# MP-Gadget/MP-Gadget

Hardware: AMD Instinct MI355X
Metric: particle-updates/sec (gravity force step: PM + tree build + short-range walk) (higher is better)
Workload: dtype f64; 1 GPU; 256^3 DM-only TreePM force step, Nmesh=512, s_zel ICs, all particles active, relative opening criterion (ErrTolForceAcc 0.002), TreeRcut 6, Asmth 1.5; particles=16777216, nmesh=512, parallelism=1 GPU

## Files before the change

### include/mpgadget_hip.h

```cpp
#ifndef MPGADGET_HIP_H
#define MPGADGET_HIP_H

#include <stddef.h>
#include <stdint.h>

#ifdef __cplusplus
extern "C" {
#endif

typedef struct mpg_engine mpg_engine;

int mpg_engine_create(mpg_engine **out, int device);
void mpg_engine_destroy(mpg_engine *eng);
const char *mpg_last_error(void);
const char *mpg_version(void);
const char *mpg_build_stamp(void);
int mpg_engine_set_stream(mpg_engine *eng, void *hip_stream);
void *mpg_engine_get_stream(mpg_engine *eng);
int mpg_engine_synchronize(mpg_engine *eng);

typedef struct mpg_gravshort_tree_params {
    double ErrTolForceAcc;
    double BHOpeningAngle;
    double MaxBHOpeningAngle;
// ... 185 lines not shown
    double density_in_phys_cgs;
    double uu_in_cgs;
    double tt_in_s;
    double units_rho_crit_baryon;
    double sfr_MinGasTemp;
    double temp_to_u;
    double HIReionTemp;
    int test_network_maxiter;
} mpg_cooling_params;
typedef struct mpg_cooling_step {
    mpg_uvbg uvbg;
    double long_mean_free_path_heating;
    double lastred[47];
    double redshift;
    double helium;
} mpg_cooling_step;
typedef struct mpg_cooling_arrays {
    const double *density;
    double *entropy;
    double *ne;
    double *sfr;
    const double *metallicity;
    const uint8_t *heiii_ionized;
    const uint8_t *tb_hydro;
} mpg_cooling_arrays;
int mpg_set_cooling_params(mpg_engine *eng, const mpg_cooling_params *par);
int mpg_set_metal_cooling_table(mpg_engine *eng, int nz, const double *zbins, int nnh, const double *nhbins, int nt, const double *tbins,
                                const double *rate);
int mpg_dev_cooling(mpg_engine *eng, const mpg_cooling_arrays *A, const mpg_sph_times *T, const mpg_cooling_step *step, const int *d_active,
                    int64_t nactive);
int mpg_cooling(mpg_engine *eng, const mpg_particle_view *pv, double BoxSize, const mpg_cooling_arrays *A, const mpg_sph_times *T,
                const mpg_cooling_step *step, const int *ActiveParticle, int64_t NumActiveParticle);
int mpg_resident_sph_cooling(mpg_engine *eng, const mpg_particle_view *pv, const mpg_sph_times *T, const mpg_cooling_step *step,
                             const int *ActiveParticle, int64_t NumActiveParticle, double *ne, const double *metallicity,
                             const uint8_t *heiii_ionized);
int mpg_dev_cooling_state(mpg_engine *eng, int64_t n, const double *d_rho, const double *d_u, double *d_ne_inout, double *d_lambdanet,
                          double *d_temp, double *d_nh0, const mpg_cooling_step *step);
int mpg_cooling_get_stats(mpg_engine *eng, int64_t stats[6]);
int mpg_cooling_export(mpg_engine *eng, int64_t n, int32_t *evaluations);

typedef struct mpg_tree_stats {
    int64_t NumParticles;
    int64_t numnodes;
    int64_t numleaves;
    int32_t maxlevel;
    double root_mass, root_cofm[3], root_hmax;
} mpg_tree_stats;
int mpg_tree_get_stats(mpg_engine *eng, mpg_tree_stats *st);
int mpg_tree_export(mpg_engine *eng, int32_t *level, double *center, double *len, double *cofm, double *mass, double *hmax,
                    int32_t *sibling, int32_t *pstart, int32_t *pcount);
int mpg_tree_export_order(mpg_engine *eng, int32_t *order);
int mpg_walk_get_counters(mpg_engine *eng, int64_t counters[10]);
int mpg_walk_get_f32_stats(mpg_engine *eng, int64_t out[2]);
typedef struct mpg_phase_times {
    float pm_deposit, pm_fft, pm_transfer, pm_readout, pm_total;
    float tree_keys, tree_sort, tree_nodes, tree_moments, tree_total;
    float walk;
    int32_t walk_launches;
} mpg_phase_times;
int mpg_get_phase_times(mpg_engine *eng, mpg_phase_times *t);
int mpg_set_instrumentation(mpg_engine *eng, int timing, int counters);
int mpg_walk_events_collect(mpg_engine *eng, double *total_ms, int *count);
int mpg_walk_events_collect2(mpg_engine *eng, double *total_ms, int *count, double *lists_ms, double *eval_ms, int *count_split);
const int *mpg_dev_tree_order(mpg_engine *eng);
int mpg_grav_short_pair(mpg_engine *eng, const mpg_particle_view *pv, const int *ActiveParticle, int64_t NumActiveParticle, double Rcut,
                        double rho0);
int mpg_dev_grav_short_pair(mpg_engine *eng, const int *d_active, int64_t nactive, double Rcut, double *d_accel, double *d_potential,
                            double rho0);

#define MPG_TIMEBINS 46
typedef struct mpg_kick_factors_s {
    double gravkick[MPG_TIMEBINS + 1];
    double hydrokick[MPG_TIMEBINS + 1];
    double dt_entr[MPG_TIMEBINS + 1];
    unsigned char bin_active[MPG_TIMEBINS + 1];
    double atime, MaxGasVel;
} mpg_kick_factors;
int mpg_dev_drift_all_particles(mpg_engine *eng, int64_t n, double *d_pos, const double *d_vel, const unsigned char *d_type,
                                const unsigned char *d_flags, double *d_hsml, const double *d_dthsml, double ddrift, double BoxSize,
                                const double random_shift[3]);
int mpg_dev_apply_pm_half_kick(mpg_engine *eng, int64_t n, double *d_vel, const double *d_gravpm, const unsigned char *d_flags, double Fgravkick);
int mpg_dev_apply_half_kick(mpg_engine *eng, int64_t n, const int *d_active, int64_t nactive, double *d_vel, const double *d_gravaccel,
                            const unsigned char *d_type, const unsigned char *d_flags, const unsigned char *d_tb_grav,
                            const unsigned char *d_tb_hydro, const double *d_hydroaccel, double *d_entropy, const double *d_dtentropy,
                            const mpg_kick_factors *K);
int mpg_dev_apply_hydro_half_kick(mpg_engine *eng, int64_t n, const int *d_active, int64_t nactive, double *d_vel, const unsigned char *d_type,
                                  const unsigned char *d_flags, const unsigned char *d_tb_hydro, const double *d_hydroaccel, double *d_entropy,
                                  const double *d_dtentropy, const mpg_kick_factors *K);

int mpg_dev_timestep_gravity_dloga(mpg_engine *eng, int64_t n, const double *d_gravaccel, const double *d_gravpm, double atime, double hubble,
                                   double ErrTolIntAccuracy, double *d_dloga);

int mpg_dev_timestep_hydro_dloga(mpg_engine *eng, int64_t n, const unsigned char *d_type, const double *d_hsml, const double *d_dthsml,
                                 const double *d_maxsignalvel, const unsigned char *d_bh_mintimebin, const double *dloga_for_bin, double atime,
                                 double hubble, double CourantFac, double *d_dloga, unsigned char *d_titype);

typedef struct {
    int64_t nsync;
    const double *loga;
} mpg_timeline;
typedef struct {
    int mintimebin, maxtimebin, mingravtimebin;
    int64_t Ti_kick[MPG_TIMEBINS + 1];
    int64_t Ti_lastactivedrift[MPG_TIMEBINS + 1];
    int64_t Ti_Current;
    int64_t PM_length, PM_start, PM_kick;
// ... 214 lines not shown
                             void **d_new_cols);
int mpg_dist_use_decomposition(mpg_dist *d, double BoxSize, double margin, int La);
int mpg_dist_domain_maintain(mpg_dist *d, int64_t n, const double *d_pos, const unsigned char *d_garbage, double BoxSize, int64_t *n_leaving);
int mpg_dist_set_domain(mpg_dist *d, double BoxSize, const mpg_topnode *TopNodes, int NTopNodes, const int *leaf_task, int NTopLeaves,
                        double margin, int La);
int mpg_dist_gravity_step(mpg_dist *d, int64_t n_own, const double *d_pos, const float *d_mass, const double *d_oldacc,
                          const double *d_prev_accel, double *d_accel, double *d_gravpm, double *d_potential, double rho0);
int mpg_dist_dev_gravpm_force(mpg_dist *d, int64_t n_own, const double *d_pos, const float *d_mass, double *d_gravpm, double *d_potential);
int mpg_dist_dev_set_types(mpg_dist *d, int64_t n_own, const uint8_t *d_type);
int mpg_dist_dev_set_garbage(mpg_dist *d, int64_t n_own, const unsigned char *d_garbage);
int mpg_dist_dev_force_tree_build(mpg_dist *d, int64_t n_own, const double *d_pos, const float *d_mass);
int mpg_dist_dev_grav_short_tree(mpg_dist *d, const double *d_oldacc, const double *d_prev_accel, const double *d_gravpm, double *d_accel,
                                 double *d_potential, double rho0);
int mpg_dist_dev_grav_short_tree_active_tree(mpg_dist *d, int64_t n_act, const double *d_pos, const float *d_mass, const double *d_oldacc,
                                             double *d_accel, double *d_potential, double rho0);
int mpg_dist_grav_short_tree_active_tree(mpg_dist *d, const mpg_particle_view *pv, const int *ActiveParticle, int64_t NumActiveParticle,
                                         double (*AccelStore)[3], double rho0);
int mpg_dist_dev_grav_short_tree_active(mpg_dist *d, const int *d_active, int64_t nactive, const double *d_oldacc, const double *d_prev_accel,
                                        const double *d_gravpm, double *d_accel, double *d_potential, double rho0);
int mpg_dist_dev_density(mpg_dist *d, int64_t n_own, const uint8_t *d_type, const mpg_sph_arrays *A, const mpg_sph_times *T, int update_hsml,
                         int DoEgyDensity);
int mpg_dist_dev_hydro_force(mpg_dist *d, int64_t n_own, const mpg_sph_arrays *A, const mpg_sph_times *T);
int mpg_dist_dev_density_active(mpg_dist *d, int64_t n_own, const uint8_t *d_type, const mpg_sph_arrays *A, const mpg_sph_times *T,
                                const int *d_active, int64_t nactive, int update_hsml, int DoEgyDensity);
int mpg_dist_dev_hydro_force_active(mpg_dist *d, int64_t n_own, const mpg_sph_arrays *A, const mpg_sph_times *T, const int *d_active,
                                    int64_t nactive);
int mpg_dist_dev_fof_fof(mpg_dist *d, int64_t n_own, const double *d_pos, const float *d_mass, const uint8_t *d_type, const uint64_t *d_id,
                         const double *d_vel, const mpg_fof_params *par, int64_t *d_grnr, int64_t *ngroups_total, int64_t *ngroups_here);
int mpg_dist_fof_groups(mpg_dist *d, const mpg_fof_groups *out);
int mpg_dist_gravpm_force(mpg_dist *d, const mpg_particle_view *pv);
int mpg_dist_force_tree_full(mpg_dist *d, const mpg_particle_view *pv);
int mpg_dist_grav_short_tree(mpg_dist *d, const mpg_particle_view *pv, double (*AccelStore)[3], double rho0);
int mpg_dist_grav_short_tree_active(mpg_dist *d, const mpg_particle_view *pv, const int *ActiveParticle, int64_t NumActiveParticle,
                                    double (*AccelStore)[3], double rho0);
int mpg_dist_set_sph_options(mpg_dist *d, int BlackHoleOn);
double mpg_dist_last_max_hsml(mpg_dist *d);
int mpg_dist_domain_set_maxpart(mpg_dist *d, int64_t MaxPart);
int mpg_dist_gravpm_get_powerspectrum(mpg_dist *d, double BoxSize_in_MPC, double *kk, double *Power, int64_t *Nmodes, int *nonzero);
int mpg_dist_potential_planes(mpg_dist *d, int64_t n_own, const double *d_pos, const float *d_mass, const uint8_t *d_type,
                              const unsigned char *d_flags, double BoxSize, const mpg_plane_params *params, double *d_planes, int64_t *npart);
int mpg_dist_density(mpg_dist *d, const mpg_particle_view *pv, const mpg_sph_arrays *A, const mpg_sph_times *T, const int *ActiveParticle,
                     int64_t NumActiveParticle, int update_hsml, int DoEgyDensity);
int mpg_dist_hydro_force(mpg_dist *d, const mpg_particle_view *pv, const mpg_sph_arrays *A, const mpg_sph_times *T, const int *ActiveParticle,
                         int64_t NumActiveParticle);
const float *mpg_dist_walk_cost(mpg_dist *d);
int mpg_dist_get_stats(mpg_dist *d, int64_t stats[8]);
int mpg_dist_get_times(mpg_dist *d, double ms[8]);
int mpg_dev_force_tree_set_min_leaf_level(mpg_engine *eng, int level);

int mpg_set_walk_threshold(mpg_engine *eng, int thresh);
int mpg_set_walk_split_mode(mpg_engine *eng, int overlap, int chunks_per_wave);
int mpg_set_walk_list_capacity(mpg_engine *eng, int cap);
int mpg_set_walk_offsets64(mpg_engine *eng, int on);
int mpg_set_walk_variant(mpg_engine *eng, int variant);
int mpg_get_walk_choice(mpg_engine *eng, int *variant, int *list_capacity, unsigned *last_overflow);

#ifdef __cplusplus
}
#endif
#endif
```

### mp-gadget_amd/csrc/engine.hip

```cpp
#include "engine_internal.h"
#include <cstdio>

static thread_local std::string g_err;
std::string &mpg_err_slot() { return g_err; }

extern "C" {

const char *mpg_last_error(void) { return g_err.c_str(); }
const char *mpg_version(void) { return "mpgadget_hip 0.1 (gfx950; TreePM gravity: PM + tree + short-range walk)"; }

int mpg_engine_create(mpg_engine **out, int device)
{
    API_BEGIN
    MPG_CHECK(out != nullptr, "mpg_engine_create: null output pointer");
    int ndev = 0;
    hipError_t e = hipGetDeviceCount(&ndev);
    if(e != hipSuccess || ndev <= 0)
        fail(__FILE__, __LINE__, "mpg_engine_create: no HIP device available (this engine has no CPU path)");
    MPG_CHECK(device >= 0 && device < ndev, "mpg_engine_create: bad device index");
    MPG_HIP(hipSetDevice(device));
    mpg_engine *eng = new mpg_engine();
    eng->device = device;
    MPG_HIP(hipStreamCreateWithFlags(&eng->stream, hipStreamNonBlocking));
    eng->own_stream = true;
// ... 1747 lines not shown
            cofm[3 * j + 0] = m[j].x;
            cofm[3 * j + 1] = m[j].y;
            cofm[3 * j + 2] = m[j].z;
        }
        if(mass)
            mass[j] = m[j].m;
        if(hmax)
            hmax[j] = hm.empty() ? 0.0 : hm[j];
    }
    API_END
}

int mpg_tree_export_order(mpg_engine *eng, int32_t *order)
{
    API_BEGIN
    MPG_CHECK(eng && order, "null argument");
    MPG_CHECK(eng->tree_allocated, "no tree");
    MPG_HIP(hipSetDevice(eng->device));
    MPG_HIP(hipStreamSynchronize(eng->stream));
    MPG_HIP(hipMemcpy(order, eng->tree.idx_b.p, eng->tree.npart * sizeof(int32_t), hipMemcpyDeviceToHost));
    API_END
}

int mpg_walk_get_counters(mpg_engine *eng, int64_t counters[10])
{
    API_BEGIN
    MPG_CHECK(eng && counters, "null argument");
    MPG_HIP(hipSetDevice(eng->device));
    MPG_HIP(hipStreamSynchronize(eng->stream));
    unsigned long long c[16] = {0};
    MPG_HIP(hipMemcpy(c, eng->counters.p, 16 * sizeof(unsigned long long), hipMemcpyDeviceToHost));
    counters[0] = (int64_t)c[0];
    counters[1] = (int64_t)c[1];
    counters[2] = (int64_t)c[2];
    counters[3] = eng->last_targets;
    for(int k = 0; k < 6; k++)
        counters[4 + k] = (int64_t)c[3 + k];
    API_END
}

int mpg_walk_get_f32_stats(mpg_engine *eng, int64_t out[2])
{
    API_BEGIN
    MPG_CHECK(eng && out, "null argument");
    MPG_HIP(hipSetDevice(eng->device));
    MPG_HIP(hipStreamSynchronize(eng->stream));
    unsigned long long c[16] = {0};
    MPG_HIP(hipMemcpy(c, eng->counters.p, 16 * sizeof(unsigned long long), hipMemcpyDeviceToHost));
    out[0] = (int64_t)c[12];
    out[1] = (int64_t)c[13];
    API_END
}

int mpg_get_phase_times(mpg_engine *eng, mpg_phase_times *t)
{
    API_BEGIN
    MPG_CHECK(eng && t, "null argument");
    *t = eng->timer.t;
    API_END
}

int mpg_set_instrumentation(mpg_engine *eng, int timing, int counters)
{
    API_BEGIN
    MPG_CHECK(eng, "null engine");
    eng->timer.enabled = timing != 0;
    eng->count = counters != 0;
    API_END
}

int mpg_walk_events_collect2(mpg_engine *eng, double *total_ms, int *count, double *lists_ms, double *eval_ms, int *count_split)
{
    API_BEGIN
    MPG_CHECK(eng && total_ms && count, "null argument");
    MPG_HIP(hipSetDevice(eng->device));
    MPG_HIP(hipStreamSynchronize(eng->stream));
    double tot = 0, tl = 0, te = 0;
    int c = 0, cs = 0;
    for(size_t k = 0; k < eng->walk_events.size(); k++) {
        auto &ev = eng->walk_events[k];
        float ms = 0;
        MPG_HIP(hipEventSynchronize(ev.second));
        MPG_HIP(hipEventElapsedTime(&ms, ev.first, ev.second));
        tot += ms;
        c++;
        if(hipEvent_t mid = k < eng->walk_mid.size() ? eng->walk_mid[k] : nullptr) {
            float a = 0, b = 0;
            MPG_HIP(hipEventElapsedTime(&a, ev.first, mid));
            MPG_HIP(hipEventElapsedTime(&b, mid, ev.second));
            tl += a;
            te += b;
            cs++;
            eng->free_mid.push_back(mid);
        }
        eng->free_events.push_back(ev);
    }
    eng->walk_events.clear();
    eng->walk_mid.clear();
    *total_ms = tot;
    *count = c;
    if(lists_ms)
        *lists_ms = tl;
    if(eval_ms)
        *eval_ms = te;
    if(count_split)
        *count_split = cs;
    API_END
}

int mpg_walk_events_collect(mpg_engine *eng, double *total_ms, int *count)
{
    return mpg_walk_events_collect2(eng, total_ms, count, nullptr, nullptr, nullptr);
}

const int *mpg_dev_tree_order(mpg_engine *eng) { return (eng && eng->tree_allocated) ? (const int *)eng->tree.idx_b.p : nullptr; }

int mpg_set_walk_split_mode(mpg_engine *eng, int overlap, int chunks_per_wave)
{
    API_BEGIN
    MPG_CHECK(eng && chunks_per_wave >= 0 && chunks_per_wave <= 1024, "bad argument");
    eng->w3.split_overlap = overlap != 0;
    eng->w3.split_chunks_per_wave = chunks_per_wave;
    API_END
}

int mpg_set_walk_offsets64(mpg_engine *eng, int on)
{
    API_BEGIN
    MPG_CHECK(eng, "null engine");
    eng->w3.split_offsets64 = on != 0;
    API_END
}

int mpg_set_walk_threshold(mpg_engine *eng, int thresh)
{
    API_BEGIN
    MPG_CHECK(eng, "null engine");
    eng->walk_thresh = thresh;
    API_END
}

int mpg_set_walk_list_capacity(mpg_engine *eng, int cap)
{
    API_BEGIN
    MPG_CHECK(eng && cap >= 16 && cap <= 65536, "walk list capacity must be in [16, 65536]");
    eng->w3.cap = cap;
    eng->w3.split_cap = (cap + 7) / 8 * 8;
    API_END
}

int mpg_get_walk_choice(mpg_engine *eng, int *variant, int *list_capacity, unsigned *last_overflow)
{
    API_BEGIN
    MPG_CHECK(eng && variant, "null argument");
    *variant = eng->walk_variant ? eng->walk_variant : eng->walk_choice;
    if(list_capacity)
        *list_capacity = eng->w3.split_cap;
    if(last_overflow)
        *last_overflow = eng->w3.split_last_overflow;
    API_END
}

int mpg_set_walk_variant(mpg_engine *eng, int variant)
{
    API_BEGIN
    MPG_CHECK(eng && (variant == 0 || variant == 1 || variant == 4 || variant == 6), "walk variant must be 0 (auto), 1, 4 or 6");
    eng->walk_variant = variant;
    eng->walk_choice = 0;
    API_END
}

}
```

### mp-gadget_amd/csrc/grav_walk.h

```cpp
#pragma once
#include "mpg_common.h"

namespace mpg {

struct WalkIO {
    int64_t ntargets = 0;
    const int *targets = nullptr;
    const double *pos = nullptr;
    const float *mass = nullptr;
    const double *oldacc = nullptr;
    const double *prev_accel = nullptr;
    const double *gravpm = nullptr;
    double *accel = nullptr;
    double *potential = nullptr;
    const float *tab_force = nullptr;
    const float *tab_pot = nullptr;
    unsigned long long *counters = nullptr;
    int list_prio = 0, eval_prio = 0;
    float *cost = nullptr;
};

void launch_grav_walk(const TreeView &tv, const GravParams &gp, const WalkIO &io, bool want_pot, bool count, bool fastwrap, int thresh,
                      hipStream_t st);

struct WalkScratch {
    DevBuf<int2> list;
    DevBuf<unsigned> ctr;
    int cap = 512;
    int num_cu = 0;
    DevBuf<unsigned> split_lists;
    DevBuf<int2> split_counts;
    DevBuf<int> split_ovf;
    int split_cap = 512;
    int split_slice = 1 << 25;
    size_t split_bytes = 80ull << 30;
    unsigned split_last_overflow = 0, split_last_maxlen = 0;
    bool split_overlap = false;
    bool split_offsets64 = false;
    int split_chunks_per_wave = 1;
    hipEvent_t ev_mid = nullptr;
    bool mid_recorded = false;
    hipEvent_t ev_before_eval = nullptr;
    hipStream_t split_stream = nullptr;
    hipEvent_t ev_lists[2] = {nullptr, nullptr}, ev_eval[2] = {nullptr, nullptr}, ev_begin = nullptr;
    ~WalkScratch()
    {
        for(hipEvent_t e : {ev_lists[0], ev_lists[1], ev_eval[0], ev_eval[1], ev_begin})
            if(e)
                (void)hipEventDestroy(e);
        if(split_stream)
            (void)hipStreamDestroy(split_stream);
    }
};
void launch_grav_walk_coop(const TreeView &tv, const GravParams &gp, const WalkIO &io, bool want_pot, bool count, bool fastwrap,
                           WalkScratch &ws, hipStream_t st);
void launch_grav_walk_split(const TreeView &tv, const GravParams &gp, const WalkIO &io, bool want_pot, bool count, bool fastwrap, WalkScratch &ws,
                            hipStream_t st);
void launch_grav_short_pair(const TreeView &tv, const GravParams &gp, const WalkIO &io, double rcut_abs, bool want_pot, unsigned *d_err,
                            hipStream_t st);
unsigned walk_coop_error(WalkScratch &ws, hipStream_t st);

}
```

### mp-gadget_amd/csrc/grav_walk_split.hip

```cpp
#include "grav_walk.h"
#include <cstdlib>
#include <cstring>
#include <cstdio>
#include <type_traits>

namespace mpg {

namespace {

constexpr int EVAL_BLOCKS = 4;
constexpr int LIST_BLOCKS = 6;

__device__ __forceinline__ double rsqrt_nr(double x)
{
    const double y = __builtin_amdgcn_rsq(x);
    const double e = fma(-(x * y), y, 1.0);
    return fma(y * e, fma(e, 0.375, 0.5), y);
}

template <unsigned long long BITS>
__device__ __forceinline__ double scalar_literal()
{
    unsigned lo, hi;
    asm volatile("s_mov_b32 %0, %2\n\ts_mov_b32 %1, %3" : "=s"(lo), "=s"(hi) : "i"((unsigned)(BITS & 0xffffffffull)), "i"((unsigned)(BITS >> 32)));
// ... 581 lines not shown
        if(tvalid) {
            const bool overflow = (overflowed >> lane) & 1u;
            if(io.cost)
                io.cost[ci] = (float)(8 * (overflow ? cap : nl) + nn + 3 * (nl + nn));
            if(overflow) {
                counts[rel] = make_int2(-1, 0);
                ovf[atomicAdd(&ctl[0], 1u)] = ci;
            }
            else {
                counts[rel] = make_int2(nl | (wrapped ? (1 << 30) : 0), nn);
                if((unsigned)(nl + nn) > ctl[2])
                    atomicMax(&ctl[2], (unsigned)(nl + nn));
            }
        }
        if(COUNT) {
#pragma unroll
            for(int t = 0; t < 8; t++)
                if(!((overflowed >> t) & 1u)) {
                    n_pp += c_pp[t];
                    if(lane == 0) {
                        n_vis += T.c_vis[t];
                        n_used += T.c_used[t];
                        n_le += (unsigned)T.nleaf[t];
                        n_se += (unsigned)T.nnode[t];
                    }
                }
        }
    }
    if(COUNT) {
        unsigned long long c0 = n_pp, c1 = n_vis, c2 = n_used, c3 = lane == 0 ? st_a : 0u, c4 = lane == 0 ? st_al : 0u;
        for(int off = 32; off > 0; off >>= 1) {
            c0 += __shfl_down(c0, off);
            c1 += __shfl_down(c1, off);
            c2 += __shfl_down(c2, off);
            c3 += __shfl_down(c3, off);
            c4 += __shfl_down(c4, off);
        }
        if(lane == 0) {
            atomicAdd(&io.counters[5], n_le);
            atomicAdd(&io.counters[6], n_se);
            atomicAdd(&io.counters[0], c0);
            atomicAdd(&io.counters[1], c1);
            atomicAdd(&io.counters[2], c2);
            atomicAdd(&io.counters[3], c3);
            atomicAdd(&io.counters[4], c4);
            if(F32 && n_amb)
                atomicAdd(&io.counters[12], (unsigned long long)n_amb);
            if(F32 && n_f32w)
                atomicAdd(&io.counters[13], (unsigned long long)n_f32w);
        }
    }
}

constexpr int RING_STRIDE = 17;

template <bool POT, bool WRAP, bool O32>
__device__ __forceinline__ void eval_lists(const TreeView &tv, const GravParams &gp, const unsigned *__restrict__ L, const int cap, const int nleaf,
                                           const int nnode, const int s, const int gshift, const double px,
                                           const double py, const double pz, const double *__restrict__ s_wtab, unsigned *__restrict__ ring_g,
                                           double &ax, double &ay, double &az, double &pot)
{
    const unsigned empty = (unsigned)tv.nnodes;
    const unsigned s32 = (unsigned)s * 32u;
#define MPG_LOAD(EJ, SV)                                                                        \
    {                                                                                           \
        const unsigned ej_ = (EJ);                                                              \
        if(O32)                                                                                 \
            SV = *(const Src4 *)((const char *)tv.srcL + (size_t)((ej_ << 8) + s32));           \
        else                                                                                    \
            SV = tv.srcL[(size_t)ej_ * 8 + (size_t)s];                                          \
    }
#define MPG_EVAL(SV)                                                              \
    {                                                                             \
        __builtin_amdgcn_sched_barrier(0);                                        \
        double dx_ = SV.x - px, dy_ = SV.y - py, dz_ = SV.z - pz;                 \
        if(WRAP) {                                                                \
            dx_ = nearest_img(dx_, gp.box, gp.invbox);                            \
            dy_ = nearest_img(dy_, gp.box, gp.invbox);                            \
            dz_ = nearest_img(dz_, gp.box, gp.invbox);                            \
        }                                                                         \
        pair_force<POT>(SV, dx_, dy_, dz_, gp, s_wtab, ax, ay, az, pot);           \
        asm volatile("" : "+v"(ax), "+v"(ay), "+v"(az), "+v"(pot));               \
        __builtin_amdgcn_sched_barrier(0);                                        \
    }
    {
        const unsigned ls = (unsigned)((gshift >> 3) * cap + s);
#define MPG_LEAF_AT(E0) (ls + (unsigned)(E0))
        __builtin_amdgcn_wave_barrier();
        ring_g[s] = (s < nleaf) ? ld<true>(L, MPG_LEAF_AT(0)) : empty;
        unsigned ent_n = (8 + s < nleaf) ? ld<true>(L, MPG_LEAF_AT(8)) : empty;
        __builtin_amdgcn_wave_barrier();
        unsigned eb = ring_g[1];
        Src4 A, B;
        MPG_LOAD(ring_g[0], A);
        int wmax = nleaf;
        for(int off = 8; off < 64; off <<= 1)
            wmax = max(wmax, __shfl_xor(wmax, off));
        wmax = __builtin_amdgcn_readfirstlane(wmax);
        Src4 Cq = A;
        MPG_LOAD(eb, B);
        int staged = 1;
#pragma unroll 1
        for(int e = 0; e < wmax; e += 3) {
            if(e + 4 >= 8 * staged) {
                ring_g[(staged & 1) * 8 + s] = ent_n;
                ent_n = ((staged + 1) * 8 + s < nleaf) ? ld<true>(L, MPG_LEAF_AT((staged + 1) * 8)) : empty;
                staged++;
                __builtin_amdgcn_wave_barrier();
            }
            const unsigned e2 = ring_g[(e + 2) & 15], e3 = ring_g[(e + 3) & 15], e4 = ring_g[(e + 4) & 15];
            MPG_LOAD(e2, Cq);
            MPG_EVAL(A);
            MPG_LOAD(e3, A);
            MPG_EVAL(B);
            MPG_LOAD(e4, B);
            MPG_EVAL(Cq);
        }
    }
    if(any_lane(nnode > 0)) {
        const unsigned NONE = (unsigned)tv.nnodes;
        const unsigned top = (unsigned)((gshift >> 3) * cap + cap - 1 - s);
#define MPG_NODE_AT(R0) (top - (unsigned)(R0))
#define MPG_NODE_ENT(R0) (((R0) + s < nnode) ? ld<true>(L, MPG_NODE_AT(R0)) : NONE)
        Src4 Sa = ld<O32>(tv.momB, MPG_NODE_ENT(0));
        Src4 Sb = ld<O32>(tv.momB, MPG_NODE_ENT(8));
        Src4 Sc;
        unsigned nx = MPG_NODE_ENT(16), ny = MPG_NODE_ENT(24), nz = MPG_NODE_ENT(32);
#pragma unroll 1
        for(int r0 = 0;; r0 += 24) {
            if(!any_lane(r0 < nnode))
                break;
            Sc = ld<O32>(tv.momB, nx);
            nx = MPG_NODE_ENT(r0 + 40);
            MPG_EVAL(Sa);
            if(!any_lane(r0 + 8 < nnode))
                break;
            Sa = ld<O32>(tv.momB, ny);
            ny = MPG_NODE_ENT(r0 + 48);
            MPG_EVAL(Sb);
            if(!any_lane(r0 + 16 < nnode))
                break;
            Sb = ld<O32>(tv.momB, nz);
            nz = MPG_NODE_ENT(r0 + 56);
            MPG_EVAL(Sc);
        }
#undef MPG_NODE_ENT
    }
#undef MPG_LOAD
#undef MPG_EVAL
#undef MPG_LEAF_AT
#undef MPG_NODE_AT
}

__device__ __attribute__((noinline)) double potential_postprocess(double pot, const double m, const double h, const double cbrtrho0, const double G)
{
    pot += m / (h / 2.8);
    pot -= 2.8372975 * pow(m, 2.0 / 3) * cbrtrho0;
    return pot * G;
}

template <bool POT, bool FASTWRAP, bool O32>
__global__ void __launch_bounds__(256, EVAL_BLOCKS) k_walk_eval(const TreeView tv, const GravParams gp, const WalkIO io, const unsigned *__restrict__ lists,
                                                    const int2 *__restrict__ counts, const int cap, const int64_t slot0, const int64_t nslots)
{
    constexpr int ROW = POT ? 4 : 2;
    __shared__ __attribute__((aligned(16))) double s_wtab[NTAB * ROW];
    __shared__ unsigned s_ring[4 * 8 * RING_STRIDE];
    set_wave_prio(io.eval_prio);
    for(int i = threadIdx.x; i < NTAB; i += blockDim.x) {
        const bool last = i == NTAB - 1;
        s_wtab[i * 2 + 0] = last ? 0.0 : (double)io.tab_force[i];
        s_wtab[i * 2 + 1] = last ? 0.0 : (double)io.tab_force[i + 1] - (double)io.tab_force[i];
        if(POT) {
            s_wtab[2 * NTAB + i * 2 + 0] = last ? 0.0 : (double)io.tab_pot[i];
            s_wtab[2 * NTAB + i * 2 + 1] = last ? 0.0 : (double)io.tab_pot[i + 1] - (double)io.tab_pot[i];
        }
    }
    __syncthreads();

    const int lane = threadIdx.x & 63;
    const int grp = lane >> 3, s = lane & 7;
    const int gshift = grp * 8;
    unsigned *__restrict__ ring_g = s_ring + ((threadIdx.x >> 6) * 8 + grp) * RING_STRIDE;
    const unsigned nchunks = (unsigned)((nslots + 7) / 8);
    const ChunkIter it(nchunks);

    for(unsigned chunk = it.lo + it.first; chunk < it.hi; chunk += it.stride) {
        const int64_t rel = (int64_t)chunk * 8 + grp;
        bool valid = rel < nslots;
        const int64_t slot = slot0 + rel;
        int ci = -1;
        double px = 0, py = 0, pz = 0;
        int nleaf = 0, nnode = 0;
        bool wrapped = false;
        if(valid) {
            const int2 c = counts[rel];
            if(c.x < 0)
                valid = false;
            else {
                nleaf = c.x & 0x3fffffff;
                wrapped = (c.x >> 30) & 1;
                nnode = c.y;
                ci = io.targets ? io.targets[slot] : tv.order[slot];
                px = io.pos[3 * (int64_t)ci + 0];
                py = io.pos[3 * (int64_t)ci + 1];
                pz = io.pos[3 * (int64_t)ci + 2];
            }
        }
        const unsigned *__restrict__ L = lists + (size_t)__builtin_amdgcn_readfirstlane((int)chunk) * (size_t)cap * 8;
        double ax = 0, ay = 0, az = 0, pot = 0;
        if(!FASTWRAP || any_lane(wrapped))
            eval_lists<POT, true, O32>(tv, gp, L, cap, nleaf, nnode, s, gshift, px, py, pz, s_wtab, ring_g, ax, ay, az, pot);
        else
            eval_lists<POT, false, O32>(tv, gp, L, cap, nleaf, nnode, s, gshift, px, py, pz, s_wtab, ring_g, ax, ay, az, pot);
        for(int off = 1; off < 8; off <<= 1) {
            ax += __shfl_xor(ax, off);
            ay += __shfl_xor(ay, off);
            az += __shfl_xor(az, off);
            if(POT)
                pot += __shfl_xor(pot, off);
        }
        if(valid && s == 0) {
            io.accel[3 * (int64_t)ci + 0] = ax * gp.G;
            io.accel[3 * (int64_t)ci + 1] = ay * gp.G;
            io.accel[3 * (int64_t)ci + 2] = az * gp.G;
            if(POT && io.potential)
                io.potential[ci] = potential_postprocess(pot, (double)io.mass[ci], gp.h, gp.cbrtrho0, gp.G);
        }
    }
}

int grid_blocks(WalkScratch &ws, const void *kern, int64_t nchunks, int chunks_per_wave)
{
    if(ws.num_cu == 0) {
        int dev = 0;
        MPG_HIP(hipGetDevice(&dev));
        MPG_HIP(hipDeviceGetAttribute(&ws.num_cu, hipDeviceAttributeMultiprocessorCount, dev));
    }
    const int64_t need = (nchunks + 3) / 4;
    int64_t nblocks;
    if(chunks_per_wave > 0)
        nblocks = (need + chunks_per_wave - 1) / chunks_per_wave;
    else {
        int occ = 0;
        MPG_HIP(hipOccupancyMaxActiveBlocksPerMultiprocessor(&occ, kern, 256, 0));
        if(occ < 1)
            occ = 1;
        if(occ > 8)
            occ = 8;
        nblocks = (int64_t)ws.num_cu * occ;
        if(nblocks > need)
            nblocks = need;
    }
    return (int)((nblocks + 7) / 8 * 8);
}

template <bool POT, bool COUNT, bool FASTWRAP, bool O32>
void launch_split_t(const TreeView &tv, const GravParams &gp, const WalkIO &io, WalkScratch &ws, hipStream_t st)
{
    const char *f32_e = getenv("MPG_LISTS_F32");
    const bool f32_env = f32_e && f32_e[0] == '1';
    const bool f32 = FASTWRAP && f32_env && gp.bhangle2 > 1e-6 && gp.bhangle2 < 1e6 && gp.rcut > 1e-12 && gp.rcut < 1e12 && gp.box < 1e12;
    auto kl = (FASTWRAP && f32) ? k_walk_lists8<COUNT, FASTWRAP, O32, FASTWRAP> : k_walk_lists8<COUNT, FASTWRAP, O32, false>;
    auto ke = k_walk_eval<POT, FASTWRAP, O32>;
    if(const char *e = getenv("MPG_LIST_CAP"))
        ws.split_cap = atoi(e) / 8 * 8;
    const int cap = ws.split_cap;
    static const size_t long_bytes = getenv("MPG_SPLIT_BYTES_LONG") ? (size_t)atoll(getenv("MPG_SPLIT_BYTES_LONG")) : ((size_t)16 << 30);
    const size_t area = cap >= 4096 ? (ws.split_bytes < long_bytes ? ws.split_bytes : long_bytes) : ws.split_bytes;
    int64_t slice = (int64_t)(area / ((size_t)cap * sizeof(unsigned))) / 2048 * 2048;
    if(slice < 65536)
        slice = 65536;
    if(slice > ws.split_slice)
        slice = ws.split_slice;
    if(const char *e = getenv("MPG_SPLIT_SLICE"))
        slice = atoll(e);
    const int64_t nmax = io.ntargets < slice ? io.ntargets : slice;
    const int64_t nslices = (io.ntargets + slice - 1) / slice;
    static const int ov_env = getenv("MPG_SPLIT_OVERLAP") ? (getenv("MPG_SPLIT_OVERLAP")[0] == '0' ? 0 : 1) : -1;
    const bool overlap = (ov_env >= 0 ? ov_env != 0 : ws.split_overlap) && nslices > 1;
    const size_t lists_sz = (size_t)((nmax + 15) / 16) * 16 * (size_t)cap, counts_sz = (size_t)nmax + 8;
    ws.split_lists.reserve(lists_sz * (overlap ? 2 : 1));
    ws.split_counts.reserve(counts_sz * (overlap ? 2 : 1));
    ws.split_ovf.reserve((size_t)io.ntargets);
    if(overlap && !ws.split_stream) {
        MPG_HIP(hipStreamCreateWithFlags(&ws.split_stream, hipStreamNonBlocking));
        for(int k = 0; k < 2; k++) {
            MPG_HIP(hipEventCreateWithFlags(&ws.ev_lists[k], hipEventDisableTiming));
            MPG_HIP(hipEventCreateWithFlags(&ws.ev_eval[k], hipEventDisableTiming));
        }
        MPG_HIP(hipEventCreateWithFlags(&ws.ev_begin, hipEventDisableTiming));
    }
    static const int cpw_env = getenv("MPG_SPLIT_CPW") ? atoi(getenv("MPG_SPLIT_CPW")) : -1;
    const int cpw = cpw_env >= 0 ? cpw_env : ws.split_chunks_per_wave;
    hipStream_t sl = overlap ? ws.split_stream : st;
    if(overlap) {
        MPG_HIP(hipEventRecord(ws.ev_begin, st));
        MPG_HIP(hipStreamWaitEvent(sl, ws.ev_begin, 0));
    }
    int64_t i = 0;
    for(int64_t s0 = 0; s0 < io.ntargets; s0 += slice, i++) {
        const int64_t ns = (io.ntargets - s0 < slice) ? io.ntargets - s0 : slice;
        const int64_t nchunks = (ns + 7) / 8;
        const int b = overlap ? (int)(i & 1) : 0;
        unsigned *lists = ws.split_lists.p + (size_t)b * lists_sz;
        int2 *counts = ws.split_counts.p + (size_t)b * counts_sz;
        if(overlap && i >= 2)
            MPG_HIP(hipStreamWaitEvent(sl, ws.ev_eval[b], 0));
        static const bool split_time = getenv("MPG_SPLIT_TIME") != nullptr;
        hipEvent_t te[3] = {nullptr, nullptr, nullptr};
        if(split_time) {
            for(auto &e : te)
                MPG_HIP(hipEventCreate(&e));
            MPG_HIP(hipEventRecord(te[0], sl));
        }
        hipLaunchKernelGGL(kl, dim3((unsigned)grid_blocks(ws, (const void *)kl, nchunks, (COUNT && cpw > 0 && cpw < 8) ? 8 : cpw)), dim3(256), 0, sl, tv, gp, io,
                           lists, counts, cap, s0, ns, ws.ctr.p, ws.split_ovf.p);
        if(split_time)
            MPG_HIP(hipEventRecord(te[1], sl));
        if(overlap) {
            MPG_HIP(hipEventRecord(ws.ev_lists[b], sl));
            MPG_HIP(hipStreamWaitEvent(st, ws.ev_lists[b], 0));
        }
        if(ws.ev_mid && nslices == 1 && !overlap) {
            MPG_HIP(hipEventRecord(ws.ev_mid, st));
            ws.mid_recorded = true;
        }
        if(ws.ev_before_eval && i == 0)
            MPG_HIP(hipStreamWaitEvent(st, ws.ev_before_eval, 0));
        hipLaunchKernelGGL(ke, dim3((unsigned)grid_blocks(ws, (const void *)ke, nchunks, cpw)), dim3(256), 0, st, tv, gp, io, lists, counts, cap, s0,
                           ns);
        if(overlap)
            MPG_HIP(hipEventRecord(ws.ev_eval[b], st));
        if(split_time) {
            MPG_HIP(hipEventRecord(te[2], st));
            MPG_HIP(hipEventSynchronize(te[2]));
            float ml = 0, me = 0;
            MPG_HIP(hipEventElapsedTime(&ml, te[0], te[1]));
            MPG_HIP(hipEventElapsedTime(&me, te[1], te[2]));
            fprintf(stderr, "SPLIT_TIME targets %lld lists %.3f ms eval %.3f ms\n", (long long)ns, ml, me);
            for(auto &e : te)
                MPG_HIP(hipEventDestroy(e));
        }
    }
    MPG_HIP(hipGetLastError());
}

}

void launch_grav_walk_split(const TreeView &tv, const GravParams &gp, const WalkIO &io, bool want_pot, bool count, bool fastwrap, WalkScratch &ws,
                            hipStream_t st)
{
    if(io.ntargets == 0)
        return;
    MPG_CHECK(tv.npart < (1ll << 29), "split walk: more than 2^29 particles in one tree");
    ws.ctr.reserve(16);
    MPG_CHECK(tv.srcL != nullptr, "split walk: the tree carries no padded leaf sources (TreeBuilder::ensure_leaf_pad)");
    const bool o32 = !ws.split_offsets64 && (tv.npart + tv.nnodes + 64) * 32 < (1ll << 32) && (tv.nnodes + 2) * 256 < (1ll << 32);
#define MPG_WS(P, C)                                                \
    do {                                                            \
        if(fastwrap) {                                              \
            if(o32)                                                 \
                launch_split_t<P, C, true, true>(tv, gp, io, ws, st);  \
            else                                                    \
                launch_split_t<P, C, true, false>(tv, gp, io, ws, st); \
        }                                                           \
        else                                                        \
            launch_split_t<P, C, false, false>(tv, gp, io, ws, st); \
    } while(0)
    unsigned ctl[4] = {0, 0, 0, 0};
    for(;;) {
        MPG_HIP(hipMemsetAsync(ws.ctr.p, 0, 16 * sizeof(unsigned), st));
        if(want_pot) {
            if(count)
                MPG_WS(true, true);
            else
                MPG_WS(true, false);
        }
        else {
            if(count)
                MPG_WS(false, true);
            else
                MPG_WS(false, false);
        }
// ... 30 lines not shown
```

### mp-gadget_amd/engine.py

```python
import ctypes as C
import os

import numpy as np

_HERE = os.path.dirname(os.path.abspath(__file__))
LIB_PATH = os.path.join(_HERE, "libmpgadget_hip.so")
TABLE_PATH = os.path.join(_HERE, "data", "shortrange_force_kernels.f64")

PARTICLE_DTYPE = np.dtype({
    "names": ["Pos", "TopLeaf", "Mass", "PI", "Flags", "TimeBinHydro", "TimeBinGravity", "Type", "Vel",
              "FullTreeGravAccel", "GravPM", "Ti_drift", "Hsml", "DtHsml", "ID", "GrNr", "Potential"],
    "formats": [("<f8", 3), "<i4", "<f4", "<i4", "u1", "u1", "u1", "u1", ("<f8", 3), ("<f8", 3), ("<f8", 3), "<i8", "<f8",
                "<f8", "<u8", "<i8", "<f8"],
    "offsets": [0, 24, 28, 32, 36, 37, 38, 39, 40, 64, 88, 112, 120, 128, 136, 144, 152],
    "itemsize": 160})

SHORTRANGE_FORCE_WINDOW_TYPE_EXACT = 0
SHORTRANGE_FORCE_WINDOW_TYPE_ERFC = 1
ALLMASK, GASMASK, DMMASK, NUMASK, STARMASK, BHMASK = 63, 1, 2, 4, 16, 32


class EngineError(RuntimeError):
    pass

# ... 237 lines not shown
            raise EngineError(self.lib.mpg_last_error().decode())

    def close(self):
        if getattr(self, "h", None):
            self.lib.mpg_engine_destroy(self.h)
            self.h = None

    def __del__(self):
        try:
            self.close()
        except Exception:
            pass

    def version(self):
        return self.lib.mpg_version().decode()

    def synchronize(self):
        self._ck(self.lib.mpg_engine_synchronize(self.h))

    def set_stream(self, raw_stream):
        self._ck(self.lib.mpg_engine_set_stream(self.h, C.c_void_p(raw_stream)))

    def use_torch_stream(self, device=None):
        import torch
        torch.cuda.synchronize()
        self._torch_stream = torch.cuda.Stream(device=device)
        torch.cuda.set_stream(self._torch_stream)
        self.set_stream(self._torch_stream.cuda_stream)
        return self._torch_stream

    def get_stream(self):
        return self.lib.mpg_engine_get_stream(self.h)

    def set_instrumentation(self, timing=True, counters=False):
        self._ck(self.lib.mpg_set_instrumentation(self.h, int(timing), int(counters)))

    def set_walk_variant(self, variant):
        self._ck(self.lib.mpg_set_walk_variant(self.h, int(variant)))

    def walk_choice(self):
        v, cap, ovf = C.c_int(0), C.c_int(0), C.c_uint(0)
        self._ck(self.lib.mpg_get_walk_choice(self.h, C.byref(v), C.byref(cap), C.byref(ovf)))
        return v.value, cap.value, ovf.value

    def set_walk_list_capacity(self, cap):
        self._ck(self.lib.mpg_set_walk_list_capacity(self.h, int(cap)))

    def set_walk_split_mode(self, overlap=True, chunks_per_wave=2):
        self._ck(self.lib.mpg_set_walk_split_mode(self.h, int(bool(overlap)), int(chunks_per_wave)))

    def set_walk_offsets64(self, on):
        self._ck(self.lib.mpg_set_walk_offsets64(self.h, int(bool(on))))

    def set_walk_threshold(self, thresh):
        self._ck(self.lib.mpg_set_walk_threshold(self.h, int(thresh)))

    def set_gravshort_treepar(self, ErrTolForceAcc=0.002, BHOpeningAngle=0.175, MaxBHOpeningAngle=0.9, TreeUseBH=2,
                              Rcut=6.0, FractionalGravitySoftening=1. / 30.):
        p = TreeParams(ErrTolForceAcc, BHOpeningAngle, MaxBHOpeningAngle, TreeUseBH, Rcut, FractionalGravitySoftening)
        self._ck(self.lib.mpg_set_gravshort_treepar(self.h, C.byref(p)))

    def get_gravshort_treepar(self):
        p = TreeParams()
        self._ck(self.lib.mpg_get_gravshort_treepar(self.h, C.byref(p)))
        return p

    def gravshort_set_softenings(self, MeanSeparation):
        self._ck(self.lib.mpg_gravshort_set_softenings(self.h, C.c_double(MeanSeparation)))

    def FORCE_SOFTENING(self):
        return self.lib.mpg_force_softening(self.h)

    def gravshort_fill_ntab(self, ShortRangeForceWindowType=SHORTRANGE_FORCE_WINDOW_TYPE_EXACT, Asmth=1.5):
        if self._table is None:
            self._table = np.fromfile(TABLE_PATH, dtype="<f8")
            if self._table.size != 512 * 5:
                raise EngineError("corrupt short-range table " + TABLE_PATH)
        self._ck(self.lib.mpg_gravshort_fill_ntab(self.h, int(ShortRangeForceWindowType), C.c_double(Asmth),
                                                  self._table.ctypes.data_as(C.c_void_p), 512))

    def gravpm_init_periodic(self, BoxSize, Asmth, Nmesh, G):
        self._ck(self.lib.mpg_gravpm_init_periodic(self.h, C.c_double(BoxSize), C.c_double(Asmth), int(Nmesh), C.c_double(G)))

    def gravpm_measure_power(self, on=True):
        self._ck(self.lib.mpg_gravpm_measure_power(self.h, int(bool(on))))

    def gravpm_get_powerspectrum(self, nmesh, BoxSize_in_MPC):
        kk, P, N = np.zeros(nmesh), np.zeros(nmesh), np.zeros(nmesh, np.int64)
        nz = C.c_int(0)
        self._ck(self.lib.mpg_gravpm_get_powerspectrum(self.h, C.c_double(BoxSize_in_MPC), kk.ctypes.data_as(C.c_void_p),
                                                       P.ctypes.data_as(C.c_void_p), N.ctypes.data_as(C.c_void_p), C.byref(nz)))
        return kk[:nz.value], P[:nz.value], N[:nz.value]

    def gravpm_set_nu_response(self, fn, BoxSize_in_MPC=1.0):
        if fn is None:
            self._ck(self.lib.mpg_gravpm_set_nu_response(self.h, None, None, C.c_double(0.0)))
            self._keep.pop("nu_response", None)
            return
        thunk = _nu_response_thunk(fn)
        self._ck(self.lib.mpg_gravpm_set_nu_response(self.h, thunk, None, C.c_double(BoxSize_in_MPC)))
        self._keep["nu_response"] = thunk

    def gravpm_nu_response_error(self):
        t = self._keep.get("nu_response")
        return None if t is None else t.error

# ... 657 lines not shown
                raise EngineError("%s must be a contiguous %s array of len(P)" % (name, want.__name__))
        s = self.cooling_step(step)
        act = None if ActiveParticle is None else np.ascontiguousarray(ActiveParticle, np.int32)
        hp = lambda t: None if t is None else C.c_void_p(t.ctypes.data)
        self._ck(self.lib.mpg_resident_sph_cooling(self.h, C.byref(v), C.byref(times), C.byref(s),
                                                   None if act is None else act.ctypes.data_as(C.c_void_p),
                                                   C.c_int64(0 if act is None else len(act)), hp(ne), hp(metallicity), hp(heiii_ionized)))

    def dev_cooling_state(self, rho, u, ne, step, lambdanet=None, temp=None, nh0=None):
        s = self.cooling_step(step)
        self._ck(self.lib.mpg_dev_cooling_state(self.h, C.c_int64(rho.shape[0]), _ptr(rho), _ptr(u), _ptr(ne), _ptr(lambdanet), _ptr(temp),
                                                _ptr(nh0), C.byref(s)))

    def cooling_stats(self):
        c = (C.c_int64 * 6)()
        self._ck(self.lib.mpg_cooling_get_stats(self.h, c))
        return dict(treated=c[0], evaluations=c[1], bisections=c[2], floor=c[3], reion=c[4], errors=c[5])

    def cooling_export(self, n):
        ev = np.zeros(n, np.int32)
        self._ck(self.lib.mpg_cooling_export(self.h, C.c_int64(n), ev.ctypes.data_as(C.c_void_p)))
        return ev

    def tree_stats(self):
        st = TreeStats()
        self._ck(self.lib.mpg_tree_get_stats(self.h, C.byref(st)))
        return st

    def tree_export(self):
        st = self.tree_stats()
        n = st.numnodes
        d = dict(level=np.zeros(n, np.int32), center=np.zeros((n, 3)), len=np.zeros(n), cofm=np.zeros((n, 3)),
                 mass=np.zeros(n), hmax=np.zeros(n), sibling=np.zeros(n, np.int32), pstart=np.zeros(n, np.int32),
                 pcount=np.zeros(n, np.int32))
        p = lambda a: a.ctypes.data_as(C.c_void_p)
        self._ck(self.lib.mpg_tree_export(self.h, p(d["level"]), p(d["center"]), p(d["len"]), p(d["cofm"]), p(d["mass"]),
                                          p(d["hmax"]), p(d["sibling"]), p(d["pstart"]), p(d["pcount"])))
        order = np.zeros(st.NumParticles, np.int32)
        self._ck(self.lib.mpg_tree_export_order(self.h, order.ctypes.data_as(C.c_void_p)))
        d["order"] = order
        return d

    def walk_counters(self):
        c = (C.c_int64 * 10)()
        self._ck(self.lib.mpg_walk_get_counters(self.h, c))
        return dict(pp=c[0], nodes_visited=c[1], nodes_used=c[2], targets=c[3], node_steps=c[4], node_lanes=c[5],
                    int_steps=c[6], int_lanes=c[7], cycles_a=c[8], cycles_b=c[9])

    def walk_f32_stats(self):
        c = (C.c_int64 * 2)()
        self._ck(self.lib.mpg_walk_get_f32_stats(self.h, c))
        return int(c[0]), int(c[1])

    def walk_events_collect(self):
        tot = C.c_double()
        cnt = C.c_int()
        self._ck(self.lib.mpg_walk_events_collect(self.h, C.byref(tot), C.byref(cnt)))
        return tot.value, cnt.value

    def walk_events_collect_split(self):
        tot, tl, te = C.c_double(), C.c_double(), C.c_double()
        cnt, cs = C.c_int(), C.c_int()
        self._ck(self.lib.mpg_walk_events_collect2(self.h, C.byref(tot), C.byref(cnt), C.byref(tl), C.byref(te), C.byref(cs)))
        return tot.value, cnt.value, tl.value, te.value, cs.value

    def dev_tree_order(self, n, device):
        import torch

        class _Holder:
            pass
        h = _Holder()
        h.__cuda_array_interface__ = {"shape": (int(n),), "typestr": "<i4", "data": (int(self.dev_tree_order_ptr()), False), "version": 2}
        return torch.as_tensor(h, device=device)

    def dev_tree_order_ptr(self):
        return self.lib.mpg_dev_tree_order(self.h)

    def phase_times(self):
        t = PhaseTimes()
        self._ck(self.lib.mpg_get_phase_times(self.h, C.byref(t)))
        return t.as_dict()


def make_particles(pos, mass, type=1):
    P = np.zeros(len(pos), dtype=PARTICLE_DTYPE)
    P["Pos"] = pos
    P["Mass"] = mass
    P["Type"] = type
    P["ID"] = np.arange(len(pos), dtype=np.uint64)
    return P
```

Measured before the change: 238.5 million particles/s.

## Sort walk targets by list length within windows to balance eval wavefronts

Adds a per-window ranking kernel that orders target slots by interaction-list length (leaf count, optionally plus node count) inside 64-slot windows. The evaluation kernel then reads slots through this permutation, so each 8-lane group in a wavefront handles targets with similar loop trip counts. This is meant to cut divergence idle time where short lists wait on the longest list in the wave. In exchange it adds a small sort kernel per slice and an indirect load, and may lose some locality from the original tree order. A counter kernel for needed versus executed steps is added for diagnostics.

```diff
diff --git a/include/mpgadget_hip.h b/include/mpgadget_hip.h
--- a/include/mpgadget_hip.h
+++ b/include/mpgadget_hip.h
@@ -261,6 +261,7 @@
 int mpg_tree_export_order(mpg_engine *eng, int32_t *order);
 int mpg_walk_get_counters(mpg_engine *eng, int64_t counters[10]);
 int mpg_walk_get_f32_stats(mpg_engine *eng, int64_t out[2]);
+int mpg_walk_get_eval_steps(mpg_engine *eng, int64_t out[2]);
 typedef struct mpg_phase_times {
     float pm_deposit, pm_fft, pm_transfer, pm_readout, pm_total;
     float tree_keys, tree_sort, tree_nodes, tree_moments, tree_total;
@@ -581,6 +582,7 @@
 int mpg_set_walk_split_mode(mpg_engine *eng, int overlap, int chunks_per_wave);
 int mpg_set_walk_list_capacity(mpg_engine *eng, int cap);
 int mpg_set_walk_offsets64(mpg_engine *eng, int on);
+int mpg_set_walk_eval_window(mpg_engine *eng, int w);
 int mpg_set_walk_variant(mpg_engine *eng, int variant);
 int mpg_get_walk_choice(mpg_engine *eng, int *variant, int *list_capacity, unsigned *last_overflow);
 
diff --git a/mp-gadget_amd/csrc/engine.hip b/mp-gadget_amd/csrc/engine.hip
--- a/mp-gadget_amd/csrc/engine.hip
+++ b/mp-gadget_amd/csrc/engine.hip
@@ -1823,6 +1823,19 @@
     API_END
 }
 
+int mpg_walk_get_eval_steps(mpg_engine *eng, int64_t out[2])
+{
+    API_BEGIN
+    MPG_CHECK(eng && out, "null argument");
+    MPG_HIP(hipSetDevice(eng->device));
+    MPG_HIP(hipStreamSynchronize(eng->stream));
+    unsigned long long c[16] = {0};
+    MPG_HIP(hipMemcpy(c, eng->counters.p, 16 * sizeof(unsigned long long), hipMemcpyDeviceToHost));
+    out[0] = (int64_t)c[14];
+    out[1] = (int64_t)c[15];
+    API_END
+}
+
 int mpg_get_phase_times(mpg_engine *eng, mpg_phase_times *t)
 {
     API_BEGIN
@@ -1903,6 +1916,15 @@
     API_END
 }
 
+int mpg_set_walk_eval_window(mpg_engine *eng, int w)
+{
+    API_BEGIN
+    MPG_CHECK(eng && (w == -1 || w == 0 || w == 64 || w == 128 || w == 256),
+              "walk evaluation window must be 0 (tree-order chunks), 64, 128, 256 or -1 (the default)");
+    eng->w3.split_eval_window = w < 0 ? WalkScratch::EVAL_WINDOW_DEFAULT : w;
+    API_END
+}
+
 int mpg_set_walk_threshold(mpg_engine *eng, int thresh)
 {
     API_BEGIN
diff --git a/mp-gadget_amd/csrc/grav_walk.h b/mp-gadget_amd/csrc/grav_walk.h
--- a/mp-gadget_amd/csrc/grav_walk.h
+++ b/mp-gadget_amd/csrc/grav_walk.h
@@ -31,6 +31,9 @@
     DevBuf<unsigned> split_lists;
     DevBuf<int2> split_counts;
     DevBuf<int> split_ovf;
+    DevBuf<int> split_perm;
+    static constexpr int EVAL_WINDOW_DEFAULT = 64;
+    int split_eval_window = EVAL_WINDOW_DEFAULT;
     int split_cap = 512;
     int split_slice = 1 << 25;
     size_t split_bytes = 80ull << 30;
diff --git a/mp-gadget_amd/csrc/grav_walk_split.hip b/mp-gadget_amd/csrc/grav_walk_split.hip
--- a/mp-gadget_amd/csrc/grav_walk_split.hip
+++ b/mp-gadget_amd/csrc/grav_walk_split.hip
@@ -657,11 +657,66 @@
     }
 }
 
+__global__ void __launch_bounds__(256) k_eval_order(const int2 *__restrict__ counts, int *__restrict__ perm, const int64_t nslots, const int sumkey)
+{
+    __shared__ unsigned s_key[256];
+    const unsigned W = blockDim.x, i = threadIdx.x;
+    const int64_t base = (int64_t)blockIdx.x * W, rel = base + i;
+    unsigned key = 0;
+    if(rel < nslots) {
+        const int2 c = counts[rel];
+        if(c.x >= 0) {
+            const unsigned nleaf = (unsigned)c.x & 0x3fffffffu;
+            const unsigned len = sumkey ? nleaf + (((unsigned)c.y + 7u) >> 3) : nleaf;
+            key = 0x80000000u | ((unsigned)c.x & 0x40000000u) | (len < 0x3fffffffu ? len : 0x3fffffffu);
+        }
+    }
+    s_key[i] = key;
+    __syncthreads();
+    unsigned rank = 0;
+    for(unsigned j = 0; j < W; j++) {
+        const unsigned k = s_key[j];
+        rank += (k > key || (k == key && j < i)) ? 1u : 0u;
+    }
+    perm[base + rank] = (int)rel;
+}
+
+__global__ void __launch_bounds__(256) k_eval_steps(const int2 *__restrict__ counts, const int *__restrict__ perm, const int64_t nslots,
+                                                    unsigned long long *__restrict__ steps)
+{
+    const int64_t chunk = (int64_t)blockIdx.x * blockDim.x + threadIdx.x;
+    unsigned long long need = 0, exec = 0;
+    if(chunk * 8 < nslots) {
+        int lmax = 0, nmax = 0;
+        for(int g = 0; g < 8; g++) {
+            const int64_t rel = perm ? (int64_t)perm[chunk * 8 + g] : chunk * 8 + g;
+            if(rel >= nslots)
+                continue;
+            const int2 c = counts[rel];
+            if(c.x < 0)
+                continue;
+            const int nleaf = c.x & 0x3fffffff, nb = (c.y + 7) >> 3;
+            need += (unsigned long long)(nleaf + nb);
+            lmax = max(lmax, nleaf);
+            nmax = max(nmax, nb);
+        }
+        exec = 8ull * (unsigned long long)((lmax + 2) / 3 * 3 + nmax);
+    }
+    for(int off = 32; off > 0; off >>= 1) {
+        need += __shfl_down(need, off);
+        exec += __shfl_down(exec, off);
+    }
+    if((threadIdx.x & 63) == 0 && exec) {
+        atomicAdd(&steps[0], need);
+        atomicAdd(&steps[1], exec);
+    }
+}
+
 constexpr int RING_STRIDE = 17;
 
 template <bool POT, bool WRAP, bool O32>
 __device__ __forceinline__ void eval_lists(const TreeView &tv, const GravParams &gp, const unsigned *__restrict__ L, const int cap, const int nleaf,
-                                           const int nnode, const int s, const int gshift, const double px,
+                                           const int nnode, const int s, const unsigned gofs, const double px,
                                            const double py, const double pz, const double *__restrict__ s_wtab, unsigned *__restrict__ ring_g,
                                            double &ax, double &ay, double &az, double &pot)
 {
@@ -689,7 +744,7 @@
         __builtin_amdgcn_sched_barrier(0);                                        \
     }
     {
-        const unsigned ls = (unsigned)((gshift >> 3) * cap + s);
+        const unsigned ls = gofs * (unsigned)cap + (unsigned)s;
 #define MPG_LEAF_AT(E0) (ls + (unsigned)(E0))
         __builtin_amdgcn_wave_barrier();
         ring_g[s] = (s < nleaf) ? ld<true>(L, MPG_LEAF_AT(0)) : empty;
@@ -724,7 +779,7 @@
     }
     if(any_lane(nnode > 0)) {
         const unsigned NONE = (unsigned)tv.nnodes;
-        const unsigned top = (unsigned)((gshift >> 3) * cap + cap - 1 - s);
+        const unsigned top = gofs * (unsigned)cap + (unsigned)(cap - 1 - s);
 #define MPG_NODE_AT(R0) (top - (unsigned)(R0))
 #define MPG_NODE_ENT(R0) (((R0) + s < nnode) ? ld<true>(L, MPG_NODE_AT(R0)) : NONE)
         Src4 Sa = ld<O32>(tv.momB, MPG_NODE_ENT(0));
@@ -766,7 +821,8 @@
 
 template <bool POT, bool FASTWRAP, bool O32>
 __global__ void __launch_bounds__(256, EVAL_BLOCKS) k_walk_eval(const TreeView tv, const GravParams gp, const WalkIO io, const unsigned *__restrict__ lists,
-                                                    const int2 *__restrict__ counts, const int cap, const int64_t slot0, const int64_t nslots)
+                                                    const int2 *__restrict__ counts, const int cap, const int64_t slot0, const int64_t nslots,
+                                                    const int *__restrict__ perm, const unsigned wmask)
 {
     constexpr int ROW = POT ? 4 : 2;
     __shared__ __attribute__((aligned(16))) double s_wtab[NTAB * ROW];
@@ -785,13 +841,14 @@
 
     const int lane = threadIdx.x & 63;
     const int grp = lane >> 3, s = lane & 7;
-    const int gshift = grp * 8;
     unsigned *__restrict__ ring_g = s_ring + ((threadIdx.x >> 6) * 8 + grp) * RING_STRIDE;
     const unsigned nchunks = (unsigned)((nslots + 7) / 8);
     const ChunkIter it(nchunks);
 
     for(unsigned chunk = it.lo + it.first; chunk < it.hi; chunk += it.stride) {
-        const int64_t rel = (int64_t)chunk * 8 + grp;
+        const unsigned pos0 = chunk * 8u, wbase = (unsigned)__builtin_amdgcn_readfirstlane((int)(pos0 & wmask));
+        const unsigned relu = perm ? (unsigned)perm[pos0 + grp] : pos0 + grp;
+        const int64_t rel = (int64_t)relu;
         bool valid = rel < nslots;
         const int64_t slot = slot0 + rel;
         int ci = -1;
@@ -812,12 +869,13 @@
                 pz = io.pos[3 * (int64_t)ci + 2];
             }
         }
-        const unsigned *__restrict__ L = lists + (size_t)__builtin_amdgcn_readfirstlane((int)chunk) * (size_t)cap * 8;
+        const unsigned *__restrict__ L = lists + (size_t)wbase * (size_t)cap;
+        const unsigned gofs = relu - wbase;
         double ax = 0, ay = 0, az = 0, pot = 0;
         if(!FASTWRAP || any_lane(wrapped))
-            eval_lists<POT, true, O32>(tv, gp, L, cap, nleaf, nnode, s, gshift, px, py, pz, s_wtab, ring_g, ax, ay, az, pot);
+            eval_lists<POT, true, O32>(tv, gp, L, cap, nleaf, nnode, s, gofs, px, py, pz, s_wtab, ring_g, ax, ay, az, pot);
         else
-            eval_lists<POT, false, O32>(tv, gp, L, cap, nleaf, nnode, s, gshift, px, py, pz, s_wtab, ring_g, ax, ay, az, pot);
+            eval_lists<POT, false, O32>(tv, gp, L, cap, nleaf, nnode, s, gofs, px, py, pz, s_wtab, ring_g, ax, ay, az, pot);
         for(int off = 1; off < 8; off <<= 1) {
             ax += __shfl_xor(ax, off);
             ay += __shfl_xor(ay, off);
@@ -888,6 +946,12 @@
     ws.split_lists.reserve(lists_sz * (overlap ? 2 : 1));
     ws.split_counts.reserve(counts_sz * (overlap ? 2 : 1));
     ws.split_ovf.reserve((size_t)io.ntargets);
+    const int W = ws.split_eval_window;
+    const size_t perm_sz = W ? (size_t)(nmax + W - 1) / W * W : 0;
+    if(W)
+        ws.split_perm.reserve(perm_sz * (overlap ? 2 : 1));
+    const char *key_e = getenv("MPG_EVAL_KEY");
+    const int sumkey = key_e && key_e[0] == '1';
     if(overlap && !ws.split_stream) {
         MPG_HIP(hipStreamCreateWithFlags(&ws.split_stream, hipStreamNonBlocking));
         for(int k = 0; k < 2; k++) {
@@ -910,6 +974,7 @@
         const int b = overlap ? (int)(i & 1) : 0;
         unsigned *lists = ws.split_lists.p + (size_t)b * lists_sz;
         int2 *counts = ws.split_counts.p + (size_t)b * counts_sz;
+        int *perm = W ? ws.split_perm.p + (size_t)b * perm_sz : nullptr;
         if(overlap && i >= 2)
             MPG_HIP(hipStreamWaitEvent(sl, ws.ev_eval[b], 0));
         static const bool split_time = getenv("MPG_SPLIT_TIME") != nullptr;
@@ -933,8 +998,12 @@
         }
         if(ws.ev_before_eval && i == 0)
             MPG_HIP(hipStreamWaitEvent(st, ws.ev_before_eval, 0));
+        if(W)
+            hipLaunchKernelGGL(k_eval_order, dim3((unsigned)((ns + W - 1) / W)), dim3((unsigned)W), 0, st, counts, perm, ns, sumkey);
         hipLaunchKernelGGL(ke, dim3((unsigned)grid_blocks(ws, (const void *)ke, nchunks, cpw)), dim3(256), 0, st, tv, gp, io, lists, counts, cap, s0,
-                           ns);
+                           ns, perm, W ? ~(unsigned)(W - 1) : ~7u);
+        if(COUNT)
+            hipLaunchKernelGGL(k_eval_steps, dim3((unsigned)((nchunks + 255) / 256)), dim3(256), 0, st, counts, perm, ns, io.counters + 14);
         if(overlap)
             MPG_HIP(hipEventRecord(ws.ev_eval[b], st));
         if(split_time) {
diff --git a/mp-gadget_amd/engine.py b/mp-gadget_amd/engine.py
--- a/mp-gadget_amd/engine.py
+++ b/mp-gadget_amd/engine.py
@@ -313,6 +313,9 @@
     def set_walk_offsets64(self, on):
         self._ck(self.lib.mpg_set_walk_offsets64(self.h, int(bool(on))))
 
+    def set_walk_eval_window(self, w=-1):
+        self._ck(self.lib.mpg_set_walk_eval_window(self.h, int(w)))
+
     def set_walk_threshold(self, thresh):
         self._ck(self.lib.mpg_set_walk_threshold(self.h, int(thresh)))
 
@@ -1076,6 +1079,11 @@
         self._ck(self.lib.mpg_walk_get_f32_stats(self.h, c))
         return int(c[0]), int(c[1])
 
+    def walk_eval_steps(self):
+        c = (C.c_int64 * 2)()
+        self._ck(self.lib.mpg_walk_get_eval_steps(self.h, c))
+        return int(c[0]), int(c[1])
+
     def walk_events_collect(self):
         tot = C.c_double()
         cnt = C.c_int()
```

Measured after the change: 231.0 million particles/s. 0.969x the previous value.
